# KevinMathewT/multimodal-propaganda-meme-classification

Measured on AMD Instinct MI355X. Metric: memes/sec (fine-tune step) ViT-B/16+BERT-base bs=32, 1/2/4/8 MI355X, higher is better.
Workload: dtype fp16

## Files before the change

include/memehip.h:

```cpp
#ifndef MEMEHIP_H
#define MEMEHIP_H

#include <stdint.h>

#ifdef __cplusplus
extern "C" {
#endif

typedef enum MhStatus {
    MH_OK = 0,
    MH_EINVAL = 1,
    MH_ESHAPE = 2,
    MH_ELAUNCH = 3
} MhStatus;

typedef void* mh_stream_t;

const char* mh_version(void);
const char* mh_status_str(int status);

#define MH_GEMM_MAX_GROUP 8
#define MH_GEMM_GELU 1
#define MH_GEMM_OUT_F32 2
#define MH_GEMM_ACCUM 4
// ... 32 lines not shown
                     int rows, int D, float eps, mh_stream_t stream);
int mh_layernorm_bwd(const void* dy , const void* x , const float* gamma,
                     const float* mean, const float* rstd, const void* dx_add ,
                     void* dx , float* part , int n_part, int rows, int D,
                     void* dx_drop ,
                     const uint32_t* rng, float drop_p, uint32_t drop_stream, mh_stream_t stream);
#define MH_LN_MAX_JOBS 4
typedef struct MhLnFwdJob {
    const void* x; const float* gamma; const float* beta; void* y; float* y_f32; float* mean; float* rstd;
    int32_t rows; float eps;
    const int32_t* rows_dev;
} MhLnFwdJob;
typedef struct MhLnBwdJob {
    const void* dy; const void* x; const float* gamma; const float* mean; const float* rstd;
    const void* dx_add; void* dx; float* part; void* dx_drop; const uint32_t* rng;
    int32_t n_part; int32_t rows; float drop_p; uint32_t drop_stream;
    const int32_t* rows_dev;
    const int32_t* drop_rows;
} MhLnBwdJob;
int mh_layernorm_fwd_grouped(const MhLnFwdJob* jobs, int n_jobs, int D, mh_stream_t stream);
int mh_layernorm_bwd_grouped(const MhLnBwdJob* jobs, int n_jobs, int D, mh_stream_t stream);
#define MH_COLSUM_MAX_JOBS 64
typedef struct MhColsumJob {
    const float* part;
    float* out0;
    float* out1;
} MhColsumJob;
int mh_colsum_partials_f32(const MhColsumJob* jobs , int n_jobs, int n_part, int D,
                           float scale, mh_stream_t stream);

int mh_attn_fwd(const void* qkv, const int64_t* key_mask, void* out, float* lse, int B, int S, int H,
                const uint32_t* rng, float drop_p, uint32_t drop_stream, mh_stream_t stream);
int mh_attn_bwd(const void* qkv, const int64_t* key_mask, const void* out, const void* dout,
                const float* lse, float* delta, void* dqkv, int B, int S, int H, const uint32_t* rng,
                float drop_p, uint32_t drop_stream, mh_stream_t stream);
int mh_attn_fwd_packed(const void* qkv, const int64_t* key_mask, void* out, float* lse, const int32_t* cu,
                       const int32_t* row_map, int B, int S, int H, const uint32_t* rng, float drop_p,
                       uint32_t drop_stream, mh_stream_t stream);
int mh_attn_bwd_packed(const void* qkv, const int64_t* key_mask, const void* out, const void* dout,
                       const float* lse, float* delta, void* dqkv, const int32_t* cu, const int32_t* row_map, int B,
                       int S, int H, const uint32_t* rng, float drop_p, uint32_t drop_stream, mh_stream_t stream);

#define MH_ATTN_MAX_GROUP 2
typedef struct MhAttnProblem {
    const void* qkv; const int64_t* key_mask; void* out; float* lse;
    const void* dout; float* delta; void* dqkv;
    const int32_t* cu; const int32_t* row_map;
    const uint32_t* rng; float drop_p; uint32_t drop_stream;
    int32_t B, S, H; int32_t reserved;
} MhAttnProblem;
int mh_attn_fwd_grouped(const MhAttnProblem* problems , int n, mh_stream_t stream);
int mh_attn_bwd_grouped(const MhAttnProblem* problems , int n, mh_stream_t stream);
int mh_attn_set_onepass(int on);

int mh_pack_plan(const int64_t* mask , int B, int S, int pool_index, int32_t* cu, int32_t* row_map,
                 int32_t* inv_map, int64_t* pmask, int32_t* pool_rows, int32_t* n_rows, mh_stream_t stream);
int mh_pack_rows(const void* src , const int32_t* row_map, const int32_t* n_rows, void* dst,
                 int max_rows, int D, mh_stream_t stream);
int mh_unpack_rows(const void* src , const int32_t* inv_map, void* dst ,
                   int max_rows, int D, mh_stream_t stream);

int mh_bert_embed_fwd(const int64_t* ids, const float* word, const float* pos, const float* type0,
                      const float* gamma, const float* beta, void* pre ,
                      void* y , float* mean, float* rstd, int B, int S, int D, int vocab,
                      float eps, const uint32_t* rng, float drop_p, uint32_t drop_stream ,
                      mh_stream_t stream);
int mh_bert_embed_bwd(const int64_t* ids, const void* d_pre , float* dword ,
                      float* dpos , float* dtype0 , int B, int S, int D,
                      int vocab, int64_t pad_id, float scale,
                      uint8_t* row_live ,
                      int32_t* first_pos , int32_t* id_count
                      ,
                      mh_stream_t stream);
int mh_image_normalize_u8(const uint8_t* src, float* dst, int B, int H, int W, const float* mean3 ,
                          const float* std3 , mh_stream_t stream);
int mh_image_resample_u8(const uint8_t* arena, const int64_t* src_off, const int32_t* hw, const int32_t* xbounds,
                         const int32_t* xcoef, int KX, const int32_t* ybounds, const int32_t* ycoef, int KY, const uint8_t* flip,
                         uint8_t* tmp, uint8_t* out, int B, int max_h, int OH, int OW, mh_stream_t stream);
int mh_image_luma_sum_u8(const uint8_t* img, unsigned long long* sums, int B, int HW, mh_stream_t stream);
int mh_image_jitter_rotate_u8(const uint8_t* in, uint8_t* scratch, uint8_t* out, const void* params, unsigned long long* lsum,
                              int B, int H, int W, mh_stream_t stream);
int mh_dropout_apply(void* x, int64_t n, const uint32_t* rng, float p, uint32_t stream_id, mh_stream_t stream);
int mh_dropout_mask_u8(uint8_t* out, int64_t n, const uint32_t* rng, float p, uint32_t stream_id,
                       mh_stream_t stream);
int mh_zero_rows_f32(const int64_t* ids, float* table, int n_ids, int D, int vocab, mh_stream_t stream);

int mh_patchify(const float* image, void* patches, int B, int C, int H, int W, int P, mh_stream_t stream);
int mh_patchify_ld(const float* image, void* patches , int B, int C, int H, int W, int P, int ld,
                   mh_stream_t stream);
int mh_copy2d_u32(const void* src, int ld_src, void* dst, int ld_dst, int rows, int cols, int pad_to, mh_stream_t stream);
int mh_vit_assemble_fwd(const void* proj , const float* cls, const float* pos,
                        void* x , int B, int Np, int D, mh_stream_t stream);
int mh_vit_assemble_bwd(const void* dx , void* dproj ,
                        float* dcls, float* dpos, int B, int Np, int D, float scale, mh_stream_t stream);

typedef struct MhHeadParams {
    const float *Wt, *bt;
    const float *Wi, *bi;
    const float *Wf, *bf_;
    const float *Wo, *bo;
} MhHeadParams;
typedef struct MhHeadGrads {
    float *Wt, *bt, *Wi, *bi, *Wf, *bf_, *Wo, *bo;
} MhHeadGrads;

int mh_head_fwd(const MhHeadParams* p , const float* text_hidden ,
// ... 185 lines not shown
```

multimodal_propaganda_meme_classification_amd/_lib.py:

```python
from __future__ import annotations

import ctypes as C
import os

_HERE = os.path.dirname(os.path.abspath(__file__))
LIB_PATH = os.path.join(_HERE, "libmemehip.so")
LIB_PATH_F16 = os.path.join(_HERE, "libmemehip_f16.so")
LIB_PATHS = {"bf16": LIB_PATH, "fp16": LIB_PATH_F16}

MH_GEMM_MAX_GROUP = 8
MH_GEMM_GELU = 1
MH_GEMM_OUT_F32 = 2
MH_GEMM_ACCUM = 4
MH_GEMM_QUICK_GELU = 8
MH_GEMM_DERIV_AUX = 16
MH_COLSUM_MAX_JOBS = 64
MH_LN_MAX_JOBS = 4
MH_ATTN_MAX_GROUP = 2

c_void_p, c_int, c_int64, c_float = C.c_void_p, C.c_int, C.c_int64, C.c_float


class MhGemmProblem(C.Structure):
    _fields_ = [("A", c_void_p), ("B", c_void_p), ("C", c_void_p), ("bias", c_void_p),
# ... 49 lines not shown
                ("min_scale", C.c_float), ("max_scale", C.c_float), ("growth_interval", C.c_int32), ("base_grad_scale", C.c_float)]


class MhLnFwdJob(C.Structure):
    _fields_ = [(n, c_void_p) for n in ("x", "gamma", "beta", "y", "y_f32", "mean", "rstd")] + \
               [("rows", C.c_int32), ("eps", C.c_float), ("rows_dev", c_void_p)]


class MhLnBwdJob(C.Structure):
    _fields_ = [(n, c_void_p) for n in ("dy", "x", "gamma", "mean", "rstd", "dx_add", "dx", "part", "dx_drop", "rng")] + \
               [("n_part", C.c_int32), ("rows", C.c_int32), ("drop_p", C.c_float), ("drop_stream", C.c_uint32),
                ("rows_dev", c_void_p), ("drop_rows", c_void_p)]


class MhAttnProblem(C.Structure):
    _fields_ = [(n, c_void_p) for n in ("qkv", "key_mask", "out", "lse", "dout", "delta", "dqkv", "cu", "row_map", "rng")] + \
               [("drop_p", C.c_float), ("drop_stream", C.c_uint32), ("B", C.c_int32), ("S", C.c_int32), ("H", C.c_int32),
                ("reserved", C.c_int32)]


class MhGemmF32(C.Structure):
    _fields_ = [("A", c_void_p), ("B", c_void_p), ("C", c_void_p), ("bias", c_void_p)] + \
               [(n, C.c_int32) for n in ("M", "N", "K", "lda", "ldb", "ldc", "flags")] + \
               [(n, c_void_p) for n in ("bn_gamma", "bn_beta", "bn_running_mean", "bn_running_var", "bn_save_mean",
                                        "bn_save_rstd", "bn_z")] + \
               [("bn_ldz", C.c_int32), ("bn_eps", C.c_float), ("bn_momentum", C.c_float), ("bn_training", C.c_int32)]


MH_F32_ACCUM, MH_F32_TANH, MH_F32_RELU, MH_F32_BN = 1, 2, 4, 8


class MhHeadParams(C.Structure):
    _fields_ = [(n, c_void_p) for n in ("Wt", "bt", "Wi", "bi", "Wf", "bf_", "Wo", "bo")]


class MhHeadGrads(C.Structure):
    _fields_ = [(n, c_void_p) for n in ("Wt", "bt", "Wi", "bi", "Wf", "bf_", "Wo", "bo")]


_PROTOS = {
    "mh_gemm_bf16_grouped": [C.POINTER(MhGemmProblem), c_int, c_int, c_int, c_void_p],
    "mh_gemm_set_trace": [c_void_p],
    "mh_gemm_ksplit_for": [c_int, c_int],
    "mh_layernorm_fwd": [c_void_p] * 7 + [c_int, c_int, c_float, c_void_p],
    "mh_layernorm_bwd": [c_void_p] * 8 + [c_int, c_int, c_int, c_void_p, c_void_p, c_float, C.c_uint32, c_void_p],
    "mh_layernorm_fwd_grouped": [C.POINTER(MhLnFwdJob), c_int, c_int, c_void_p],
    "mh_layernorm_bwd_grouped": [C.POINTER(MhLnBwdJob), c_int, c_int, c_void_p],
    "mh_colsum_partials_f32": [C.POINTER(MhColsumJob), c_int, c_int, c_int, c_float, c_void_p],
    "mh_attn_fwd": [c_void_p] * 4 + [c_int, c_int, c_int, c_void_p, c_float, C.c_uint32, c_void_p],
    "mh_attn_bwd": [c_void_p] * 7 + [c_int, c_int, c_int, c_void_p, c_float, C.c_uint32, c_void_p],
    "mh_attn_fwd_grouped": [C.POINTER(MhAttnProblem), c_int, c_void_p],
    "mh_attn_bwd_grouped": [C.POINTER(MhAttnProblem), c_int, c_void_p],
    "mh_attn_set_onepass": [c_int],
    "mh_attn_fwd_packed": [c_void_p] * 6 + [c_int, c_int, c_int, c_void_p, c_float, C.c_uint32, c_void_p],
    "mh_attn_bwd_packed": [c_void_p] * 9 + [c_int, c_int, c_int, c_void_p, c_float, C.c_uint32, c_void_p],
    "mh_pack_plan": [c_void_p, c_int, c_int, c_int] + [c_void_p] * 6 + [c_void_p],
    "mh_pack_rows": [c_void_p] * 4 + [c_int, c_int, c_void_p],
    "mh_unpack_rows": [c_void_p] * 3 + [c_int, c_int, c_void_p],
    "mh_bert_embed_fwd": [c_void_p] * 10 + [c_int, c_int, c_int, c_int, c_float, c_void_p, c_float, C.c_uint32, c_void_p],
    "mh_image_normalize_u8": [c_void_p, c_void_p, c_int, c_int, c_int, C.POINTER(c_float), C.POINTER(c_float), c_void_p],
    "mh_image_resample_u8": [c_void_p] * 5 + [c_int] + [c_void_p] * 2 + [c_int] + [c_void_p] * 3 + [c_int] * 4 + [c_void_p],
    "mh_image_luma_sum_u8": [c_void_p, c_void_p, c_int, c_int, c_void_p],
    "mh_image_jitter_rotate_u8": [c_void_p] * 5 + [c_int] * 3 + [c_void_p],
    "mh_dropout_apply": [c_void_p, c_int64, c_void_p, c_float, C.c_uint32, c_void_p],
    "mh_dropout_mask_u8": [c_void_p, c_int64, c_void_p, c_float, C.c_uint32, c_void_p],
    "mh_bert_embed_bwd": [c_void_p] * 5 + [c_int, c_int, c_int, c_int, c_int64, c_float, c_void_p, c_void_p, c_void_p, c_void_p],
    "mh_zero_rows_f32": [c_void_p, c_void_p, c_int, c_int, c_int, c_void_p],
    "mh_patchify": [c_void_p, c_void_p] + [c_int] * 5 + [c_void_p],
    "mh_patchify_ld": [c_void_p, c_void_p] + [c_int] * 6 + [c_void_p],
    "mh_copy2d_u32": [c_void_p, c_int, c_void_p, c_int, c_int, c_int, c_int, c_void_p],
    "mh_vit_assemble_fwd": [c_void_p] * 4 + [c_int] * 3 + [c_void_p],
    "mh_vit_assemble_bwd": [c_void_p] * 4 + [c_int] * 3 + [c_float, c_void_p],
    "mh_head_fwd": [C.POINTER(MhHeadParams), c_void_p, c_void_p, c_int] + [c_void_p] * 4 + [c_int] * 7 + [c_void_p, c_float, C.c_uint32, c_void_p, c_void_p],
    "mh_head_bwd": [C.POINTER(MhHeadParams), C.POINTER(MhHeadGrads)] + [c_void_p] * 8 + [c_int] * 8 + [c_float, c_void_p, c_float, C.c_uint32, c_void_p, c_void_p],
    "mh_pool_fwd": [c_void_p, c_void_p, c_int, c_void_p] + [c_int] * 5 + [c_void_p, c_void_p],
    "mh_pool_bwd": [c_void_p, c_void_p, c_void_p, c_int] + [c_int] * 5 + [c_float, c_void_p, c_void_p],
    "mh_bn1d_fwd": [c_void_p, c_int, c_void_p, c_void_p, c_void_p, c_void_p, c_void_p, c_int, c_void_p, c_void_p, c_int, c_int,
                    c_float, c_float, c_int, c_int, c_void_p],
    "mh_bn1d_bwd": [c_void_p, c_int, c_void_p, c_int, c_void_p, c_int, c_void_p, c_void_p, c_void_p, c_void_p, c_int, c_void_p,
                    c_void_p, c_int, c_int, c_int, c_void_p],
    "mh_gemm_f32": [C.POINTER(MhGemmF32), c_int, c_int, c_void_p],
    "mh_colsum_f32": [c_void_p, c_int, c_void_p, c_int, c_int, c_float, c_void_p],
    "mh_pool_max_fwd": [c_void_p, c_void_p, c_void_p, c_int, c_int, c_int, c_void_p],
    "mh_pool_max_bwd": [c_void_p, c_void_p, c_void_p, c_int, c_int, c_int, c_void_p],
    "mh_pool_mean_fwd": [c_void_p, c_void_p, c_void_p, c_int, c_int, c_int, c_void_p],
    "mh_pool_mean_bwd": [c_void_p, c_void_p, c_void_p, c_int, c_int, c_int, c_void_p],
    "mh_pool_attn_fwd": [c_void_p] * 7 + [c_int] * 4 + [c_void_p],
    "mh_pool_attn_bwd": [c_void_p] * 9 + [c_int] * 4 + [c_void_p],
    "mh_pad_seq_f32": [c_void_p, c_void_p] + [c_int] * 5 + [c_void_p],
    "mh_relu_max_fwd": [c_void_p, c_void_p, c_void_p] + [c_int] * 4 + [c_void_p],
    "mh_relu_max_bwd": [c_void_p, c_void_p, c_void_p] + [c_int] * 3 + [c_void_p],
    "mh_conv_fold_f32": [c_void_p, c_void_p] + [c_int] * 7 + [c_void_p],
    "mh_mca3_fwd": [c_void_p] * 9 + [c_int, c_int, c_void_p],
    "mh_mca3_bwd": [c_void_p] * 15 + [c_int, c_int, c_void_p],
    "mh_softmax_gate_fwd": [c_void_p, c_void_p, c_void_p, c_int, c_int, c_void_p],
    "mh_softmax_gate_bwd": [c_void_p] * 5 + [c_int, c_int, c_void_p],
    "mh_nchw_to_nhwc": [c_void_p, c_void_p] + [c_int] * 5 + [c_void_p],
    "mh_im2col_nhwc": [c_void_p, c_void_p] + [c_int] * 9 + [c_void_p],
    "mh_col2im_nhwc": [c_void_p, c_void_p] + [c_int] * 9 + [c_void_p],
    "mh_conv_weight_pack": [c_void_p, c_void_p] + [c_int] * 6 + [c_void_p],
    "mh_conv_weight_unpack": [c_void_p, c_void_p] + [c_int] * 6 + [c_float, c_void_p],
    "mh_conv_weight_pack_batched": [C.POINTER(MhConvPackJob), c_int, c_void_p],
    "mh_conv_wgrad_finish_batched": [C.POINTER(MhConvWgradJob), c_int, c_void_p],
    "mh_conv_splitk": [C.POINTER(MhConvGeom), c_int],
    "mh_conv_fwd": [c_void_p, c_void_p, c_void_p, c_void_p, c_void_p, C.POINTER(MhConvGeom), c_void_p],
    "mh_conv_dgrad": [c_void_p, c_void_p, c_void_p, c_void_p, C.POINTER(MhConvGeom), C.POINTER(MhConvBnBwd), c_void_p],
# ... 73 lines not shown
```

multimodal_propaganda_meme_classification_amd/csrc/attention.hip:

```cpp
#include "common.h"
#include <stdlib.h>

namespace {

constexpr int HD = 64;
constexpr int TILE = 64;
constexpr int IMG = TILE * HD * 2;
constexpr float NEG_BIG = -1.0e30f;
constexpr float LOG2E = 1.4426950408889634f;
constexpr float LN2 = 0.6931471805599453f;

MH_DEV int row_img_off(int row, int chunk) { return row * 128 + ((chunk ^ ((row ^ (row >> 3)) & 7)) << 4); }
MH_DEV int tr_img_off(int row, int unit) { return row * 128 + ((unit ^ (((row >> 1) & 1) << 1)) << 5); }

template <int NT>
struct TileRegs {
    static constexpr int CH = (TILE * 8 + NT - 1) / NT;
    i32x4 v[CH];
};
template <int NT>
MH_DEV void tile_load(const h16* __restrict__ base, size_t pitch, int row0, int nrows, int tid, TileRegs<NT>& R) {
#pragma unroll
    for (int i = 0; i < TileRegs<NT>::CH; ++i) {
        const int q = tid + i * NT;
// ... 676 lines not shown
    extern __shared__ __attribute__((aligned(16))) char smem[];
    attn_bwd_dkv_body<NW, NT_RES, DROP>(A, blockIdx.x, gridDim.x, blockIdx.y, smem);
}
template <int RES_A, bool DROP_B>
__global__ __launch_bounds__(448) void attn_fwd_dual_kernel(const AttnArgs A, const AttnArgs Bp, const int nA) {
    extern __shared__ __attribute__((aligned(16))) char smem[];
    if ((int)blockIdx.y < nA) {
        attn_fwd_body<7, RES_A, false>(A, 0, 1, blockIdx.y, smem);
    } else {
        if (threadIdx.x >= 256) return;
        attn_fwd_body<4, 2, DROP_B>(Bp, 0, 1, blockIdx.y - nA, smem);
    }
}
template <bool DROP_B>
__global__ __launch_bounds__(448) void attn_bwd_dq_dual_kernel(const AttnArgs A, const AttnArgs Bp, const int nA) {
    extern __shared__ __attribute__((aligned(16))) char smem[];
    if ((int)blockIdx.y < nA) {
        attn_bwd_dq_body<7, 0, false>(A, 0, 1, blockIdx.y, smem);
    } else {
        if (threadIdx.x >= 256) return;
        attn_bwd_dq_body<4, 2, DROP_B>(Bp, 0, 1, blockIdx.y - nA, smem);
    }
}
template <bool DROP_B>
__global__ __launch_bounds__(448) void attn_bwd_dkv_dual_kernel(const AttnArgs A, const AttnArgs Bp, const int nA) {
    extern __shared__ __attribute__((aligned(16))) char smem[];
    if ((int)blockIdx.y < nA) {
        attn_bwd_dkv_body<7, 0, false>(A, 0, 1, blockIdx.y, smem);
    } else {
        if (threadIdx.x >= 256) return;
        attn_bwd_dkv_body<4, 2, DROP_B>(Bp, 0, 1, blockIdx.y - nA, smem);
    }
}

template <int RES_B, bool DROP_B>
__global__ __launch_bounds__(448) void attn_bwd_merged_dual_kernel(const AttnArgs A, const AttnArgs Bp, const int nA,
                                                                   const int nB) {
    extern __shared__ __attribute__((aligned(16))) char smem[];
    const int y = blockIdx.y;
    if (y < nA) {
        attn_bwd_dq_body<7, 0, false>(A, 0, 1, y, smem);
    } else if (y < 2 * nA) {
        attn_bwd_dkv_body<7, 0, false, true>(A, 0, 1, y - nA, smem);
    } else {
        if (threadIdx.x >= 256) return;
        if (y < 2 * nA + nB) attn_bwd_dq_body<4, RES_B, DROP_B>(Bp, 0, 1, y - 2 * nA, smem);
        else attn_bwd_dkv_body<4, RES_B, DROP_B, true>(Bp, 0, 1, y - 2 * nA - nB, smem);
    }
}


constexpr int OP_NB = 7, OP_ROWS = OP_NB * 32, OP_IMG = OP_ROWS * 128;
constexpr int OP_MB_PITCH = 72, OP_MB = 32 * OP_MB_PITCH;
constexpr int OP_LDS = 5 * OP_IMG + OP_NB * OP_MB + 2 * OP_ROWS * 4;

MH_DEV void attn_bwd_onepass_body(const AttnArgs& A, const int bh, char* smem) {
    const h16* __restrict__ qkv = A.qkv;
    const h16* __restrict__ outp = A.out;
    const h16* __restrict__ dout = A.dout;
    const float* __restrict__ lse = A.lse;
    float* __restrict__ delta = A.delta;
    h16* __restrict__ dqkv = A.dqkv;
    const int S = A.S, H = A.H;
    const int b = bh / H, hh = bh % H;
    const int tid = threadIdx.x, lane = tid & 63, wave = tid >> 6, h = lane >> 5;
    const size_t pitch = (size_t)3 * H * HD;
    const size_t r0 = (size_t)b * S;
    const int Sb = S;
    const h16* qb = qkv + r0 * pitch + hh * HD;
    const h16* kb = qb + (size_t)H * HD;
    const h16* vb = qb + (size_t)2 * H * HD;
    const h16* dob = dout + r0 * H * HD + hh * HD;
    const float c = 0.125f * LOG2E;

    char* q_img = smem;
    char* qt_img = smem + OP_IMG;
    char* do_img = smem + 2 * OP_IMG;
    char* dot_img = smem + 3 * OP_IMG;
    char* kt_img = smem + 4 * OP_IMG;
    char* mbox = smem + 5 * OP_IMG;
    float* lse_t = (float*)(mbox + OP_NB * OP_MB);
    float* dl_t = lse_t + OP_ROWS;

    {
        const uint32_t qk_bytes = (uint32_t)(((size_t)(Sb - 1) * pitch + HD) * 2);
        const uint32_t do_bytes = (uint32_t)(((size_t)(Sb - 1) * H * HD + HD) * 2);
        const __amdgpu_buffer_rsrc_t rq = mh_rsrc(qb, qk_bytes), rk = mh_rsrc(kb, qk_bytes), rd = mh_rsrc(dob, do_bytes);
        const int uw = __builtin_amdgcn_readfirstlane(wave);
#pragma unroll
        for (int i = 0; i < OP_ROWS / 8 / OP_NB; ++i) {
            const int p = uw + i * OP_NB;
            const int r = p * 8 + (lane >> 3), cp = lane & 7;
            const int c_row = cp ^ ((r ^ (r >> 3)) & 7);
            const int c_tr = ((((cp >> 1) ^ (((r >> 1) & 1) << 1)) << 1) | (cp & 1));
            const uint32_t oq = (uint32_t)r * (uint32_t)pitch * 2u, od = (uint32_t)r * (uint32_t)(H * HD) * 2u;
            char* dst = smem + p * 1024;
            __builtin_amdgcn_raw_ptr_buffer_load_lds(rq, LDS_PTR(void, dst), 16, oq + c_row * 16, 0, 0, 0);
            __builtin_amdgcn_raw_ptr_buffer_load_lds(rq, LDS_PTR(void, dst + OP_IMG), 16, oq + c_tr * 16, 0, 0, 0);
            __builtin_amdgcn_raw_ptr_buffer_load_lds(rd, LDS_PTR(void, dst + 2 * OP_IMG), 16, od + c_row * 16, 0, 0, 0);
            __builtin_amdgcn_raw_ptr_buffer_load_lds(rd, LDS_PTR(void, dst + 3 * OP_IMG), 16, od + c_tr * 16, 0, 0, 0);
            __builtin_amdgcn_raw_ptr_buffer_load_lds(rk, LDS_PTR(void, dst + 4 * OP_IMG), 16, oq + c_tr * 16, 0, 0, 0);
        }
    }
    const int wk0 = wave * 32;
    const bool mine = wk0 < Sb;
    h16x8 kf[4], vf[4];
    load_rows_frag(kb, pitch, wk0, Sb, lane, kf);
    load_rows_frag(vb, pitch, wk0, Sb, lane, vf);
    {
        const int i = tid >> 1, hf = tid & 1;
        float dl = 0.f;
        if (i < Sb) {
            const h16* dr = dob + (size_t)i * H * HD + 8 * hf;
            const h16* orow = outp + (r0 + i) * (size_t)H * HD + hh * HD + 8 * hf;
#pragma unroll
            for (int s4 = 0; s4 < 4; ++s4) {
                Pack8 a, o;
                a.v = *(const i32x4*)(dr + 16 * s4);
                o.v = *(const i32x4*)(orow + 16 * s4);
#pragma unroll
                for (int j = 0; j < 8; ++j) dl += (float)a.h[j] * (float)o.h[j];
            }
        }
        dl += mh_xor_partner<1>(dl, 0u);
        if (hf == 0) {
            dl_t[i] = dl;
            lse_t[i] = i < Sb ? lse[((size_t)b * H + hh) * S + i] * LOG2E : 1.0e30f;
            if (i < Sb) delta[((size_t)b * H + hh) * S + i] = dl;
        }
    }
    __syncthreads();

    const float kbias = (wk0 + (lane & 31)) < Sb ? 0.f : NEG_BIG;
    f32x16 dk[2], dv[2], dq[2];
#pragma unroll
    for (int i = 0; i < 2; ++i)
#pragma unroll
        for (int g = 0; g < 16; ++g) { dk[i][g] = 0.f; dv[i][g] = 0.f; dq[i][g] = 0.f; }

    for (int j = 0; j < OP_NB; ++j) {
        int qblk = wave + j;
        if (qblk >= OP_NB) qblk -= OP_NB;
        const int q0 = qblk * 32;
        if (mine && q0 < Sb) {
            f32x16 st, dp;
#pragma unroll
            for (int g = 0; g < 16; ++g) { st[g] = 0.f; dp[g] = 0.f; }
#pragma unroll
            for (int s = 0; s < 4; ++s) {
                st = MH_MFMA_32x32x16(frag_rows(q_img, q0, s, lane), kf[s], st, 0, 0, 0);
                dp = MH_MFMA_32x32x16(frag_rows(do_img, q0, s, lane), vf[s], dp, 0, 0, 0);
            }
            f32x16 pp;
#pragma unroll
            for (int g4 = 0; g4 < 4; ++g4) {
                const f32x4 l4 = *(const f32x4*)(lse_t + q0 + 8 * g4 + 4 * h);
                const f32x4 d4 = *(const f32x4*)(dl_t + q0 + 8 * g4 + 4 * h);
#pragma unroll
                for (int e = 0; e < 4; ++e) {
                    const int g = 4 * g4 + e;
                    const float pr = __builtin_amdgcn_exp2f(st[g] * c + kbias - l4[e]);
                    pp[g] = pr;
                    st[g] = pr * (dp[g] - d4[e]);
                }
            }
#pragma unroll
            for (int s = 0; s < 2; ++s) {
                const h16x8 pf = acc_frag(pp, s);
                const h16x8 df = acc_frag(st, s);
#pragma unroll
                for (int dt = 0; dt < 2; ++dt) {
                    dv[dt] = MH_MFMA_32x32x16(frag_tr(dot_img, q0, s, dt * 32, lane), pf, dv[dt], 0, 0, 0);
                    dk[dt] = MH_MFMA_32x32x16(frag_tr(qt_img, q0, s, dt * 32, lane), df, dk[dt], 0, 0, 0);
                }
            }
            char* mb = mbox + qblk * OP_MB + (lane & 31) * 2;
#pragma unroll
            for (int g4 = 0; g4 < 4; ++g4)
#pragma unroll
                for (int e = 0; e < 4; ++e) *(h16*)(mb + (8 * g4 + 4 * h + e) * OP_MB_PITCH) = (h16)st[4 * g4 + e];
        }
        __syncthreads();
        int src = wave - j;
        if (src < 0) src += OP_NB;
        if (mine && src * 32 < Sb) {
            const char* mb = mbox + wave * OP_MB + (lane & 31) * OP_MB_PITCH;
#pragma unroll
            for (int s = 0; s < 2; ++s) {
                union {
                    struct { i32x2 lo, hi; } v;
                    h16x8 f;
                } u;
                u.v.lo = *(const i32x2*)(mb + (16 * s + 4 * h) * 2);
                u.v.hi = *(const i32x2*)(mb + (16 * s + 8 + 4 * h) * 2);
#pragma unroll
                for (int dt = 0; dt < 2; ++dt)
                    dq[dt] = MH_MFMA_32x32x16(frag_tr(kt_img, src * 32, s, dt * 32, lane), u.f, dq[dt], 0, 0, 0);
            }
        }
        __syncthreads();
    }
    if (!mine) return;
    store_rows_from_T(dqkv + r0 * pitch + hh * HD, pitch, wk0, Sb, lane, dq, 0.125f);
    store_rows_from_T(dqkv + r0 * pitch + (size_t)H * HD + hh * HD, pitch, wk0, Sb, lane, dk, 0.125f);
    store_rows_from_T(dqkv + r0 * pitch + (size_t)2 * H * HD + hh * HD, pitch, wk0, Sb, lane, dv, 1.0f);
}

__global__ __launch_bounds__(448) void attn_bwd_onepass_kernel(const AttnArgs A) {
    extern __shared__ __attribute__((aligned(16))) char smem[];
    attn_bwd_onepass_body(A, blockIdx.x, smem);
}
template <int RES_B, bool DROP_B>
__global__ __launch_bounds__(448) void attn_bwd_onepass_dual_kernel(const AttnArgs A, const AttnArgs Bp, const int nA, const int nB) {
    extern __shared__ __attribute__((aligned(16))) char smem[];
    const int y = blockIdx.y;
    if (y < nA) {
        attn_bwd_onepass_body(A, y, smem);
    } else {
        if (threadIdx.x >= 256) return;
        if (y < nA + nB) attn_bwd_dq_body<4, RES_B, DROP_B>(Bp, 0, 1, y - nA, smem);
        else attn_bwd_dkv_body<4, RES_B, DROP_B, true>(Bp, 0, 1, y - nA - nB, smem);
    }
}
template <int RES_B, bool DROP_B>
__global__ __launch_bounds__(256) void attn_bwd_merged_single_kernel(const AttnArgs Bp, const int nB) {
    extern __shared__ __attribute__((aligned(16))) char smem[];
    const int y = blockIdx.y;
    if (y < nB) attn_bwd_dq_body<4, RES_B, DROP_B>(Bp, 0, 1, y, smem);
    else attn_bwd_dkv_body<4, RES_B, DROP_B, true>(Bp, 0, 1, y - nB, smem);
}

template <typename K>
void set_lds(K kern, int bytes) {
    (void)hipFuncSetAttribute((const void*)kern, hipFuncAttributeMaxDynamicSharedMemorySize, bytes);
}
int bwd_resident_max() {
    static int v = -1;
    if (v < 0) {
        const char* e = getenv("MEMEHIP_ATTN_BWD_RESIDENT_MAX");
        v = e ? atoi(e) : 128;
    }
    return v;
}
int bwd_merged_mode() {
    static int v = -1;
    if (v < 0) {
        const char* e = getenv("MEMEHIP_ATTN_BWD_MERGED");
        v = e ? atoi(e) : 2;
        if (v < 0 || v > 2) v = 2;
    }
    return v;
}
bool seven_waves() {
    static int v = -1;
    if (v < 0) {
        const char* e = getenv("MEMEHIP_ATTN_SEVEN_WAVES");
        v = e ? atoi(e) : 1;
    }
    return v != 0;
}
bool fwd_seven_waves() {
    static int v = -1;
    if (v < 0) {
        const char* e = getenv("MEMEHIP_ATTN_FWD_SEVEN_WAVES");
        v = e ? atoi(e) : 1;
    }
    return v != 0;
}
int g_onepass = -1;
bool onepass_on() {
    if (g_onepass < 0) {
        const char* e = getenv("MEMEHIP_ATTN_ONEPASS");
        g_onepass = e ? atoi(e) : 2;
    }
    return g_onepass != 0;
}
int split_for(int S) {
    const int tiles32 = (S + 31) / 32;
    return tiles32 > 4 ? 2 : 1;
}

}

#define ATTN_LAUNCH(KERN, NW_, NT_, GRID, LDS, ARGS)                                                      \
    do {                                                                                                 \
        if (dr) {                                                                                        \
            static bool once_t = (set_lds(KERN<NW_, NT_, true>, LDS), true);                             \
            (void)once_t;                                                                                \
            hipLaunchKernelGGL((KERN<NW_, NT_, true>), GRID, dim3(NW_ * 64), LDS, s, ARGS);              \
        } else {                                                                                         \
            static bool once_f = (set_lds(KERN<NW_, NT_, false>, LDS), true);                            \
            (void)once_f;                                                                                \
            hipLaunchKernelGGL((KERN<NW_, NT_, false>), GRID, dim3(NW_ * 64), LDS, s, ARGS);             \
        }                                                                                                \
    } while (0)
#define ATTN_LAUNCH_DUAL(KERN, LDS, GRID, A_, B_, NA_)                                                   \
    do {                                                                                                 \
        if (dr) {                                                                                        \
            static bool once_t = (set_lds(KERN<true>, LDS), true);                                       \
            (void)once_t;                                                                                \
            hipLaunchKernelGGL((KERN<true>), GRID, dim3(448), LDS, s, A_, B_, NA_);                      \
        } else {                                                                                         \
            static bool once_f = (set_lds(KERN<false>, LDS), true);                                      \
            (void)once_f;                                                                                \
            hipLaunchKernelGGL((KERN<false>), GRID, dim3(448), LDS, s, A_, B_, NA_);                     \
        }                                                                                                \
    } while (0)

namespace {

int check_problem(const MhAttnProblem& p, bool bwd) {
    if (!p.qkv || !p.out || !p.lse) return MH_EINVAL;
    if (bwd && (!p.dout || !p.delta || !p.dqkv)) return MH_EINVAL;
    if (p.B < 1 || p.S < 1 || p.H < 1 || p.drop_p < 0.f || p.drop_p >= 1.f) return MH_ESHAPE;
    return MH_OK;
}
AttnArgs to_args(const MhAttnProblem& p) {
    AttnArgs a;
    a.qkv = (const h16*)p.qkv;
    a.key_mask = p.key_mask;
    a.out = (h16*)p.out;
    a.lse = p.lse;
    a.dout = (const h16*)p.dout;
    a.delta = p.delta;
    a.dqkv = (h16*)p.dqkv;
    a.B = p.B; a.S = p.S; a.H = p.H;
    a.rng = p.rng; a.drop_p = p.drop_p; a.drop_stream = p.drop_stream;
    a.cu = p.cu; a.row_map = p.row_map;
    return a;
}
bool has_drop(const MhAttnProblem& p) { return p.rng && p.drop_p > 0.f; }

constexpr int lds_fwd(int nt) { return 2 * (nt > 0 ? nt : 1) * IMG + 2 * (nt > 0 ? nt : 1) * TILE * 4 + 64; }
constexpr int lds_dq(int nt) { return 3 * (nt > 0 ? nt : 1) * IMG + 2 * (nt > 0 ? nt : 1) * TILE * 4 + 64; }
constexpr int lds_dkv(int nt) { return 4 * (nt > 0 ? nt : 1) * IMG + 3 * (nt > 0 ? nt : 1) * TILE * 4; }
constexpr int cmax(int a, int b) { return a > b ? a : b; }

void launch_fwd(const MhAttnProblem& p, hipStream_t s) {
    const AttnArgs a = to_args(p);
    const bool dr = has_drop(p);
    const int S = p.S, BH = p.B * p.H;
    if (S <= 128) ATTN_LAUNCH(attn_fwd_kernel, 4, 2, dim3(split_for(S), BH), lds_fwd(2), a);
    else if (S <= 224 && fwd_seven_waves()) ATTN_LAUNCH(attn_fwd_kernel, 7, 4, dim3(1, BH), lds_fwd(4), a);
    else if (S <= 256) ATTN_LAUNCH(attn_fwd_kernel, 4, 4, dim3(split_for(S), BH), lds_fwd(4), a);
    else ATTN_LAUNCH(attn_fwd_kernel, 4, 0, dim3((S + 127) / 128, BH), lds_fwd(0), a);
}

bool onepass_fits(const MhAttnProblem& p) {
    return onepass_on() && p.S > 128 && p.S <= OP_ROWS && !p.key_mask && !p.cu && !has_drop(p);
}
void launch_onepass(const AttnArgs& a, int BH, hipStream_t s) {
    static bool once = (set_lds(attn_bwd_onepass_kernel, OP_LDS), true);
    (void)once;
    hipLaunchKernelGGL(attn_bwd_onepass_kernel, dim3(BH), dim3(448), OP_LDS, s, a);
}

void launch_bwd(const MhAttnProblem& p, hipStream_t s) {
    const AttnArgs a = to_args(p);
    const bool dr = has_drop(p);
    const int S = p.S, BH = p.B * p.H;
    const int rmax = bwd_resident_max();
    if (onepass_fits(p)) {
        launch_onepass(a, BH, s);
        return;
    }
    if (S <= 128 && S <= rmax) {
        const dim3 grid(split_for(S), BH);
        ATTN_LAUNCH(attn_bwd_dq_kernel, 4, 2, grid, lds_dq(2), a);
        ATTN_LAUNCH(attn_bwd_dkv_kernel, 4, 2, grid, lds_dkv(2), a);
    } else if (S <= 256 && S <= rmax) {
        const dim3 grid(split_for(S), BH);
        ATTN_LAUNCH(attn_bwd_dq_kernel, 4, 4, grid, lds_dq(4), a);
        ATTN_LAUNCH(attn_bwd_dkv_kernel, 4, 4, grid, lds_dkv(4), a);
    } else if (S > 128 && S <= 224 && seven_waves()) {
        const dim3 grid(1, BH);
        ATTN_LAUNCH(attn_bwd_dq_kernel, 7, 0, grid, lds_dq(0), a);
        ATTN_LAUNCH(attn_bwd_dkv_kernel, 7, 0, grid, lds_dkv(0), a);
    } else {
        const dim3 grid((S + 127) / 128, BH);
        ATTN_LAUNCH(attn_bwd_dq_kernel, 4, 0, grid, lds_dq(0), a);
        ATTN_LAUNCH(attn_bwd_dkv_kernel, 4, 0, grid, lds_dkv(0), a);
    }
}

bool dual_off() {
    static int v = -1;
    if (v < 0) {
        const char* e = getenv("MEMEHIP_ATTN_DUAL");
        v = (e && atoi(e) == 0) ? 1 : 0;
    }
    return v != 0;
}
bool dual_pair(const MhAttnProblem* p, int n, int& ia, int& ib) {
    if (n != 2 || dual_off() || !seven_waves() || !fwd_seven_waves() || bwd_resident_max() < 128) return false;
    for (int k = 0; k < 2; ++k) {
        const MhAttnProblem &a = p[k], &b = p[1 - k];
        if (a.S > 128 && a.S <= 224 && !has_drop(a) && b.S <= 128) {
            ia = k;
            ib = 1 - k;
            return true;
        }
    }
    return false;
}

}

extern "C" int mh_attn_fwd_grouped(const MhAttnProblem* p, int n, mh_stream_t stream) {
    if (!p || n < 1 || n > MH_ATTN_MAX_GROUP) return MH_EINVAL;
    for (int i = 0; i < n; ++i)
        if (int st = check_problem(p[i], false)) return st;
    hipStream_t s = (hipStream_t)stream;
    int ia, ib;
    if (dual_pair(p, n, ia, ib)) {
        const AttnArgs A = to_args(p[ia]), Bp = to_args(p[ib]);
        const int nA = p[ia].B * p[ia].H, nB = p[ib].B * p[ib].H;
        const bool dr = has_drop(p[ib]);
        constexpr int L = cmax(lds_fwd(4), lds_fwd(2));
        if (dr) {
            static bool once_t = (set_lds(attn_fwd_dual_kernel<4, true>, L), true);
            (void)once_t;
            hipLaunchKernelGGL((attn_fwd_dual_kernel<4, true>), dim3(1, nA + nB), dim3(448), L, s, A, Bp, nA);
        } else {
            static bool once_f = (set_lds(attn_fwd_dual_kernel<4, false>, L), true);
            (void)once_f;
            hipLaunchKernelGGL((attn_fwd_dual_kernel<4, false>), dim3(1, nA + nB), dim3(448), L, s, A, Bp, nA);
        }
    } else {
        for (int i = 0; i < n; ++i) launch_fwd(p[i], s);
    }
    return mh_launch_status();
}

extern "C" int mh_attn_bwd_grouped(const MhAttnProblem* p, int n, mh_stream_t stream) {
    if (!p || n < 1 || n > MH_ATTN_MAX_GROUP) return MH_EINVAL;
    for (int i = 0; i < n; ++i)
        if (int st = check_problem(p[i], true)) return st;
    hipStream_t s = (hipStream_t)stream;
    int ia, ib;
    if (dual_pair(p, n, ia, ib)) {
        const AttnArgs A = to_args(p[ia]), Bp = to_args(p[ib]);
        const int nA = p[ia].B * p[ia].H, nB = p[ib].B * p[ib].H;
        const bool dr = has_drop(p[ib]);
        const int mode = bwd_merged_mode();
        if (onepass_fits(p[ia])) {
            constexpr int L = cmax(lds_dq(2), lds_dkv(2));
            if (g_onepass == 2) {
                if (dr) {
                    static bool o7 = (set_lds(attn_bwd_onepass_dual_kernel<2, true>, OP_LDS), true);
                    (void)o7;
                    hipLaunchKernelGGL((attn_bwd_onepass_dual_kernel<2, true>), dim3(1, nA + 2 * nB), dim3(448), OP_LDS, s, A, Bp, nA, nB);
                } else {
                    static bool o8 = (set_lds(attn_bwd_onepass_dual_kernel<2, false>, OP_LDS), true);
                    (void)o8;
                    hipLaunchKernelGGL((attn_bwd_onepass_dual_kernel<2, false>), dim3(1, nA + 2 * nB), dim3(448), OP_LDS, s, A, Bp, nA, nB);
                }
                return mh_launch_status();
            }
            launch_onepass(A, nA, s);
            if (dr) {
                static bool o5 = (set_lds(attn_bwd_merged_single_kernel<2, true>, L), true);
                (void)o5;
                hipLaunchKernelGGL((attn_bwd_merged_single_kernel<2, true>), dim3(1, 2 * nB), dim3(256), L, s, Bp, nB);
            } else {
                static bool o6 = (set_lds(attn_bwd_merged_single_kernel<2, false>, L), true);
                (void)o6;
                hipLaunchKernelGGL((attn_bwd_merged_single_kernel<2, false>), dim3(1, 2 * nB), dim3(256), L, s, Bp, nB);
            }
        } else if (mode == 0) {
            const dim3 grid(1, nA + nB);
            ATTN_LAUNCH_DUAL(attn_bwd_dq_dual_kernel, cmax(lds_dq(0), lds_dq(2)), grid, A, Bp, nA);
            ATTN_LAUNCH_DUAL(attn_bwd_dkv_dual_kernel, cmax(lds_dkv(0), lds_dkv(2)), grid, A, Bp, nA);
        } else {
            const dim3 grid(1, 2 * (nA + nB));
            if (mode == 2) {
                constexpr int L = cmax(cmax(lds_dq(0), lds_dkv(0)), cmax(lds_dq(2), lds_dkv(2)));
                if (dr) {
                    static bool o1 = (set_lds(attn_bwd_merged_dual_kernel<2, true>, L), true);
                    (void)o1;
                    hipLaunchKernelGGL((attn_bwd_merged_dual_kernel<2, true>), grid, dim3(448), L, s, A, Bp, nA, nB);
                } else {
                    static bool o2 = (set_lds(attn_bwd_merged_dual_kernel<2, false>, L), true);
                    (void)o2;
                    hipLaunchKernelGGL((attn_bwd_merged_dual_kernel<2, false>), grid, dim3(448), L, s, A, Bp, nA, nB);
                }
            } else {
                constexpr int L = cmax(lds_dq(0), lds_dkv(0));
                if (dr) {
                    static bool o3 = (set_lds(attn_bwd_merged_dual_kernel<0, true>, L), true);
                    (void)o3;
                    hipLaunchKernelGGL((attn_bwd_merged_dual_kernel<0, true>), grid, dim3(448), L, s, A, Bp, nA, nB);
                } else {
                    static bool o4 = (set_lds(attn_bwd_merged_dual_kernel<0, false>, L), true);
                    (void)o4;
                    hipLaunchKernelGGL((attn_bwd_merged_dual_kernel<0, false>), grid, dim3(448), L, s, A, Bp, nA, nB);
                }
            }
        }
    } else {
        for (int i = 0; i < n; ++i) launch_bwd(p[i], s);
    }
    return mh_launch_status();
}

extern "C" int mh_attn_set_onepass(int on) {
    g_onepass = on;
    return MH_OK;
}

static MhAttnProblem one_problem(const void* qkv, const int64_t* key_mask, const void* out, float* lse, const void* dout,
                                 float* delta, void* dqkv, const int32_t* cu, const int32_t* row_map, int B, int S, int H,
                                 const uint32_t* rng, float drop_p, uint32_t drop_stream) {
    MhAttnProblem p;
    p.qkv = qkv; p.key_mask = key_mask; p.out = (void*)out; p.lse = lse;
    p.dout = dout; p.delta = delta; p.dqkv = dqkv;
    p.cu = cu; p.row_map = row_map;
    p.rng = rng; p.drop_p = drop_p; p.drop_stream = drop_stream;
    p.B = B; p.S = S; p.H = H; p.reserved = 0;
    return p;
}

extern "C" int mh_attn_fwd(const void* qkv, const int64_t* key_mask, void* out, float* lse, int B, int S,
                           int H, const uint32_t* rng, float drop_p, uint32_t drop_stream, mh_stream_t stream) {
    const MhAttnProblem p = one_problem(qkv, key_mask, out, lse, nullptr, nullptr, nullptr, nullptr, nullptr, B, S, H, rng,
                                        drop_p, drop_stream);
    return mh_attn_fwd_grouped(&p, 1, stream);
}
extern "C" int mh_attn_fwd_packed(const void* qkv, const int64_t* key_mask, void* out, float* lse, const int32_t* cu,
                                  const int32_t* row_map, int B, int S, int H, const uint32_t* rng, float drop_p,
                                  uint32_t drop_stream, mh_stream_t stream) {
    if (!cu) return MH_EINVAL;
    const MhAttnProblem p = one_problem(qkv, key_mask, out, lse, nullptr, nullptr, nullptr, cu, row_map, B, S, H, rng,
                                        drop_p, drop_stream);
    return mh_attn_fwd_grouped(&p, 1, stream);
}
extern "C" int mh_attn_bwd(const void* qkv, const int64_t* key_mask, const void* out, const void* dout,
                           const float* lse, float* delta, void* dqkv, int B, int S, int H, const uint32_t* rng,
                           float drop_p, uint32_t drop_stream, mh_stream_t stream) {
    const MhAttnProblem p = one_problem(qkv, key_mask, out, (float*)lse, dout, delta, dqkv, nullptr, nullptr, B, S, H, rng,
                                        drop_p, drop_stream);
    return mh_attn_bwd_grouped(&p, 1, stream);
}
extern "C" int mh_attn_bwd_packed(const void* qkv, const int64_t* key_mask, const void* out, const void* dout,
                                  const float* lse, float* delta, void* dqkv, const int32_t* cu, const int32_t* row_map,
                                  int B, int S, int H, const uint32_t* rng, float drop_p, uint32_t drop_stream,
                                  mh_stream_t stream) {
    if (!cu) return MH_EINVAL;
    const MhAttnProblem p = one_problem(qkv, key_mask, out, (float*)lse, dout, delta, dqkv, cu, row_map, B, S, H, rng,
                                        drop_p, drop_stream);
    return mh_attn_bwd_grouped(&p, 1, stream);
}
```

Before: 3311.

## Add one-pass attention backward for short text sequences with key masking

Templates the one-pass attention backward body on block count and a TEXT mode, so BERT text heads (S<=128, no dropout) compute dQ/dK/dV in a single kernel, with per-wave key-mask bias and skipping of fully masked key blocks. Packed variable-length sequences are handled through cu offsets. A new dual kernel runs ViT one-pass heads and text one-pass heads in one launch, replacing the separate dq/dkv merged kernel for text. The feature is on by default behind an env toggle. It adds LDS-size coupling and uses 256-thread blocks inside a 448-thread launch.

```diff
diff --git a/include/memehip.h b/include/memehip.h
--- a/include/memehip.h
+++ b/include/memehip.h
@@ -108,6 +108,7 @@
 int mh_attn_fwd_grouped(const MhAttnProblem* problems , int n, mh_stream_t stream);
 int mh_attn_bwd_grouped(const MhAttnProblem* problems , int n, mh_stream_t stream);
 int mh_attn_set_onepass(int on);
+int mh_attn_set_text_onepass(int on);
 
 int mh_pack_plan(const int64_t* mask , int B, int S, int pool_index, int32_t* cu, int32_t* row_map,
                  int32_t* inv_map, int64_t* pmask, int32_t* pool_rows, int32_t* n_rows, mh_stream_t stream);
diff --git a/multimodal_propaganda_meme_classification_amd/_lib.py b/multimodal_propaganda_meme_classification_amd/_lib.py
--- a/multimodal_propaganda_meme_classification_amd/_lib.py
+++ b/multimodal_propaganda_meme_classification_amd/_lib.py
@@ -125,6 +125,7 @@
     "mh_attn_fwd_grouped": [C.POINTER(MhAttnProblem), c_int, c_void_p],
     "mh_attn_bwd_grouped": [C.POINTER(MhAttnProblem), c_int, c_void_p],
     "mh_attn_set_onepass": [c_int],
+    "mh_attn_set_text_onepass": [c_int],
     "mh_attn_fwd_packed": [c_void_p] * 6 + [c_int, c_int, c_int, c_void_p, c_float, C.c_uint32, c_void_p],
     "mh_attn_bwd_packed": [c_void_p] * 9 + [c_int, c_int, c_int, c_void_p, c_float, C.c_uint32, c_void_p],
     "mh_pack_plan": [c_void_p, c_int, c_int, c_int] + [c_void_p] * 6 + [c_void_p],
diff --git a/multimodal_propaganda_meme_classification_amd/csrc/attention.hip b/multimodal_propaganda_meme_classification_amd/csrc/attention.hip
--- a/multimodal_propaganda_meme_classification_amd/csrc/attention.hip
+++ b/multimodal_propaganda_meme_classification_amd/csrc/attention.hip
@@ -752,21 +752,29 @@
 
 constexpr int OP_NB = 7, OP_ROWS = OP_NB * 32, OP_IMG = OP_ROWS * 128;
 constexpr int OP_MB_PITCH = 72, OP_MB = 32 * OP_MB_PITCH;
-constexpr int OP_LDS = 5 * OP_IMG + OP_NB * OP_MB + 2 * OP_ROWS * 4;
-
+constexpr int op_lds(int nb, bool text) { return 5 * nb * 32 * 128 + nb * OP_MB + 2 * nb * 32 * 4 + (text ? nb * 4 : 0); }
+constexpr int OP_LDS = op_lds(OP_NB, false);
+constexpr int OPT_NB = 4, OPT_LDS = op_lds(OPT_NB, true);
+
+template <int NB, bool TEXT>
 MH_DEV void attn_bwd_onepass_body(const AttnArgs& A, const int bh, char* smem) {
+    constexpr int ROWS = NB * 32, IMGB = ROWS * 128;
     const h16* __restrict__ qkv = A.qkv;
+    const int64_t* __restrict__ key_mask = A.key_mask;
     const h16* __restrict__ outp = A.out;
     const h16* __restrict__ dout = A.dout;
     const float* __restrict__ lse = A.lse;
     float* __restrict__ delta = A.delta;
     h16* __restrict__ dqkv = A.dqkv;
+    const int32_t* __restrict__ cu = A.cu;
     const int S = A.S, H = A.H;
     const int b = bh / H, hh = bh % H;
     const int tid = threadIdx.x, lane = tid & 63, wave = tid >> 6, h = lane >> 5;
     const size_t pitch = (size_t)3 * H * HD;
-    const size_t r0 = (size_t)b * S;
-    const int Sb = S;
+    const size_t r0 = (TEXT && cu) ? (size_t)cu[b] : (size_t)b * S;
+    const int Sb = (TEXT && cu) ? cu[b + 1] - cu[b] : S;
+    if (TEXT && Sb <= 0) return;
+    const int nb = TEXT ? (Sb + 31) / 32 : NB;
     const h16* qb = qkv + r0 * pitch + hh * HD;
     const h16* kb = qb + (size_t)H * HD;
     const h16* vb = qb + (size_t)2 * H * HD;
@@ -774,13 +782,14 @@
     const float c = 0.125f * LOG2E;
 
     char* q_img = smem;
-    char* qt_img = smem + OP_IMG;
-    char* do_img = smem + 2 * OP_IMG;
-    char* dot_img = smem + 3 * OP_IMG;
-    char* kt_img = smem + 4 * OP_IMG;
-    char* mbox = smem + 5 * OP_IMG;
-    float* lse_t = (float*)(mbox + OP_NB * OP_MB);
-    float* dl_t = lse_t + OP_ROWS;
+    char* qt_img = smem + IMGB;
+    char* do_img = smem + 2 * IMGB;
+    char* dot_img = smem + 3 * IMGB;
+    char* kt_img = smem + 4 * IMGB;
+    char* mbox = smem + 5 * IMGB;
+    float* lse_t = (float*)(mbox + NB * OP_MB);
+    float* dl_t = lse_t + ROWS;
+    int* kany = (int*)(dl_t + ROWS);
 
     {
         const uint32_t qk_bytes = (uint32_t)(((size_t)(Sb - 1) * pitch + HD) * 2);
@@ -788,18 +797,19 @@
         const __amdgpu_buffer_rsrc_t rq = mh_rsrc(qb, qk_bytes), rk = mh_rsrc(kb, qk_bytes), rd = mh_rsrc(dob, do_bytes);
         const int uw = __builtin_amdgcn_readfirstlane(wave);
 #pragma unroll
-        for (int i = 0; i < OP_ROWS / 8 / OP_NB; ++i) {
-            const int p = uw + i * OP_NB;
+        for (int i = 0; i < ROWS / 8 / NB; ++i) {
+            const int p = uw + i * NB;
+            if (TEXT && p >= 4 * nb) continue;
             const int r = p * 8 + (lane >> 3), cp = lane & 7;
             const int c_row = cp ^ ((r ^ (r >> 3)) & 7);
             const int c_tr = ((((cp >> 1) ^ (((r >> 1) & 1) << 1)) << 1) | (cp & 1));
             const uint32_t oq = (uint32_t)r * (uint32_t)pitch * 2u, od = (uint32_t)r * (uint32_t)(H * HD) * 2u;
             char* dst = smem + p * 1024;
             __builtin_amdgcn_raw_ptr_buffer_load_lds(rq, LDS_PTR(void, dst), 16, oq + c_row * 16, 0, 0, 0);
-            __builtin_amdgcn_raw_ptr_buffer_load_lds(rq, LDS_PTR(void, dst + OP_IMG), 16, oq + c_tr * 16, 0, 0, 0);
-            __builtin_amdgcn_raw_ptr_buffer_load_lds(rd, LDS_PTR(void, dst + 2 * OP_IMG), 16, od + c_row * 16, 0, 0, 0);
-            __builtin_amdgcn_raw_ptr_buffer_load_lds(rd, LDS_PTR(void, dst + 3 * OP_IMG), 16, od + c_tr * 16, 0, 0, 0);
-            __builtin_amdgcn_raw_ptr_buffer_load_lds(rk, LDS_PTR(void, dst + 4 * OP_IMG), 16, oq + c_tr * 16, 0, 0, 0);
+            __builtin_amdgcn_raw_ptr_buffer_load_lds(rq, LDS_PTR(void, dst + IMGB), 16, oq + c_tr * 16, 0, 0, 0);
+            __builtin_amdgcn_raw_ptr_buffer_load_lds(rd, LDS_PTR(void, dst + 2 * IMGB), 16, od + c_row * 16, 0, 0, 0);
+            __builtin_amdgcn_raw_ptr_buffer_load_lds(rd, LDS_PTR(void, dst + 3 * IMGB), 16, od + c_tr * 16, 0, 0, 0);
+            __builtin_amdgcn_raw_ptr_buffer_load_lds(rk, LDS_PTR(void, dst + 4 * IMGB), 16, oq + c_tr * 16, 0, 0, 0);
         }
     }
     const int wk0 = wave * 32;
@@ -807,6 +817,13 @@
     h16x8 kf[4], vf[4];
     load_rows_frag(kb, pitch, wk0, Sb, lane, kf);
     load_rows_frag(vb, pitch, wk0, Sb, lane, vf);
+    float kbias_t = NEG_BIG;
+    if (TEXT) {
+        const int key = wk0 + (lane & 31);
+        if (key < Sb && (!key_mask || key_mask[r0 + key] != 0)) kbias_t = 0.f;
+        const bool any = __ballot(kbias_t == 0.f) != 0ull;
+        if (lane == 0) kany[wave] = any;
+    }
     {
         const int i = tid >> 1, hf = tid & 1;
         float dl = 0.f;
@@ -831,18 +848,19 @@
     }
     __syncthreads();
 
-    const float kbias = (wk0 + (lane & 31)) < Sb ? 0.f : NEG_BIG;
+    const float kbias = TEXT ? kbias_t : (wk0 + (lane & 31)) < Sb ? 0.f : NEG_BIG;
+    const bool sends = mine && (!TEXT || __builtin_amdgcn_readfirstlane(kany[wave]) != 0);
     f32x16 dk[2], dv[2], dq[2];
 #pragma unroll
     for (int i = 0; i < 2; ++i)
 #pragma unroll
         for (int g = 0; g < 16; ++g) { dk[i][g] = 0.f; dv[i][g] = 0.f; dq[i][g] = 0.f; }
 
-    for (int j = 0; j < OP_NB; ++j) {
+    for (int j = 0; j < nb; ++j) {
         int qblk = wave + j;
-        if (qblk >= OP_NB) qblk -= OP_NB;
+        if (qblk >= nb) qblk -= nb;
         const int q0 = qblk * 32;
-        if (mine && q0 < Sb) {
+        if (sends && q0 < Sb) {
             f32x16 st, dp;
 #pragma unroll
             for (int g = 0; g < 16; ++g) { st[g] = 0.f; dp[g] = 0.f; }
@@ -882,8 +900,8 @@
         }
         __syncthreads();
         int src = wave - j;
-        if (src < 0) src += OP_NB;
-        if (mine && src * 32 < Sb) {
+        if (src < 0) src += nb;
+        if (mine && src * 32 < Sb && (!TEXT || __builtin_amdgcn_readfirstlane(kany[src]) != 0)) {
             const char* mb = mbox + wave * OP_MB + (lane & 31) * OP_MB_PITCH;
 #pragma unroll
             for (int s = 0; s < 2; ++s) {
@@ -908,18 +926,32 @@
 
 __global__ __launch_bounds__(448) void attn_bwd_onepass_kernel(const AttnArgs A) {
     extern __shared__ __attribute__((aligned(16))) char smem[];
-    attn_bwd_onepass_body(A, blockIdx.x, smem);
+    attn_bwd_onepass_body<OP_NB, false>(A, blockIdx.x, smem);
+}
+__global__ __launch_bounds__(256) void attn_bwd_onepass_text_kernel(const AttnArgs A) {
+    extern __shared__ __attribute__((aligned(16))) char smem[];
+    attn_bwd_onepass_body<OPT_NB, true>(A, blockIdx.x, smem);
 }
 template <int RES_B, bool DROP_B>
 __global__ __launch_bounds__(448) void attn_bwd_onepass_dual_kernel(const AttnArgs A, const AttnArgs Bp, const int nA, const int nB) {
     extern __shared__ __attribute__((aligned(16))) char smem[];
     const int y = blockIdx.y;
     if (y < nA) {
-        attn_bwd_onepass_body(A, y, smem);
+        attn_bwd_onepass_body<OP_NB, false>(A, y, smem);
     } else {
         if (threadIdx.x >= 256) return;
         if (y < nA + nB) attn_bwd_dq_body<4, RES_B, DROP_B>(Bp, 0, 1, y - nA, smem);
         else attn_bwd_dkv_body<4, RES_B, DROP_B, true>(Bp, 0, 1, y - nA - nB, smem);
+    }
+}
+__global__ __launch_bounds__(448) void attn_bwd_onepass2_dual_kernel(const AttnArgs A, const AttnArgs Bp, const int nA) {
+    extern __shared__ __attribute__((aligned(16))) char smem[];
+    const int y = blockIdx.y;
+    if (y < nA) {
+        attn_bwd_onepass_body<OP_NB, false>(A, y, smem);
+    } else {
+        if (threadIdx.x >= OPT_NB * 64) return;
+        attn_bwd_onepass_body<OPT_NB, true>(Bp, y - nA, smem);
     }
 }
 template <int RES_B, bool DROP_B>
@@ -974,6 +1006,14 @@
         g_onepass = e ? atoi(e) : 2;
     }
     return g_onepass != 0;
+}
+int g_text_onepass = -1;
+bool text_onepass_on() {
+    if (g_text_onepass < 0) {
+        const char* e = getenv("MEMEHIP_ATTN_TEXT_ONEPASS");
+        g_text_onepass = e ? atoi(e) : 1;
+    }
+    return g_text_onepass != 0;
 }
 int split_for(int S) {
     const int tiles32 = (S + 31) / 32;
@@ -1055,6 +1095,13 @@
     hipLaunchKernelGGL(attn_bwd_onepass_kernel, dim3(BH), dim3(448), OP_LDS, s, a);
 }
 
+bool text_onepass_fits(const MhAttnProblem& p) { return text_onepass_on() && p.S <= OPT_NB * 32 && !has_drop(p); }
+void launch_onepass_text(const AttnArgs& a, int BH, hipStream_t s) {
+    static bool once = (set_lds(attn_bwd_onepass_text_kernel, OPT_LDS), true);
+    (void)once;
+    hipLaunchKernelGGL(attn_bwd_onepass_text_kernel, dim3(BH), dim3(OPT_NB * 64), OPT_LDS, s, a);
+}
+
 void launch_bwd(const MhAttnProblem& p, hipStream_t s) {
     const AttnArgs a = to_args(p);
     const bool dr = has_drop(p);
@@ -1062,6 +1109,10 @@
     const int rmax = bwd_resident_max();
     if (onepass_fits(p)) {
         launch_onepass(a, BH, s);
+        return;
+    }
+    if (text_onepass_fits(p)) {
+        launch_onepass_text(a, BH, s);
         return;
     }
     if (S <= 128 && S <= rmax) {
@@ -1145,6 +1196,13 @@
         const int mode = bwd_merged_mode();
         if (onepass_fits(p[ia])) {
             constexpr int L = cmax(lds_dq(2), lds_dkv(2));
+            if (g_onepass == 2 && text_onepass_fits(p[ib])) {
+                static_assert(OPT_LDS <= OP_LDS, "the text heads run with the ViT heads' LDS");
+                static bool o9 = (set_lds(attn_bwd_onepass2_dual_kernel, OP_LDS), true);
+                (void)o9;
+                hipLaunchKernelGGL(attn_bwd_onepass2_dual_kernel, dim3(1, nA + nB), dim3(448), OP_LDS, s, A, Bp, nA);
+                return mh_launch_status();
+            }
             if (g_onepass == 2) {
                 if (dr) {
                     static bool o7 = (set_lds(attn_bwd_onepass_dual_kernel<2, true>, OP_LDS), true);
@@ -1158,7 +1216,9 @@
                 return mh_launch_status();
             }
             launch_onepass(A, nA, s);
-            if (dr) {
+            if (text_onepass_fits(p[ib])) {
+                launch_onepass_text(Bp, nB, s);
+            } else if (dr) {
                 static bool o5 = (set_lds(attn_bwd_merged_single_kernel<2, true>, L), true);
                 (void)o5;
                 hipLaunchKernelGGL((attn_bwd_merged_single_kernel<2, true>), dim3(1, 2 * nB), dim3(256), L, s, Bp, nB);
@@ -1207,6 +1267,10 @@
     g_onepass = on;
     return MH_OK;
 }
+extern "C" int mh_attn_set_text_onepass(int on) {
+    g_text_onepass = on;
+    return MH_OK;
+}
 
 static MhAttnProblem one_problem(const void* qkv, const int64_t* key_mask, const void* out, float* lse, const void* dout,
                                  float* delta, void* dqkv, const int32_t* cu, const int32_t* row_map, int B, int S, int H,
```

New measurement: 3308 (median of 6 runs). No clear change (-0.1%).
